# yanglei18/SGV3D

Hardware: AMD Instinct MI355X
Metric: camera frames/sec at 864x1536->BEV (higher is better)
Workload: dtype f32

## Files before the change

include/sgv3d_hip.h:

```cpp
#ifndef SGV3D_HIP_H
#define SGV3D_HIP_H

#include <stddef.h>
#include <stdint.h>

#ifdef __cplusplus
extern "C" {
#endif

#define SGV3D_OK 0
#define SGV3D_EINVAL (-1)
#define SGV3D_ELAUNCH (-2)
#define SGV3D_ENOSPACE (-3)

const char *sgv3d_last_error(void);
int sgv3d_abi_version(void);


int sgv3d_voxel_pooling_forward(int batch_size, int num_points, int num_channels,
                                int num_voxel_x, int num_voxel_y, int num_voxel_z,
                                const int32_t *geom_xyz, const float *input_features,
                                float *output_features, int32_t *pos_memo, void *stream);
int sgv3d_voxel_pooling_forward_fresh(int batch_size, int num_points, int num_channels,
                                      int num_voxel_x, int num_voxel_y, int num_voxel_z,
// ... 226 lines not shown

int sgv3d_deform_im2col3x3(int batch, int h, int w, int channels, int groups, const float *x,
                           const float *offset, int off_ld, float *col, void *stream);

int sgv3d_head_final_conv(int batch, int h, int w, int num_branches, int hidden_ch, int total_out,
                          const float *hidden, const float *weight, const float *bias,
                          const int32_t *branch_of_out, float *out, void *stream);

size_t sgv3d_centerhead_branches_workspace_bytes(int batch, int h, int w, int total_out);
int sgv3d_centerhead_branches_forward(int batch, int h, int w, int cin, int x_ld, int x_coff, const float *x,
                                      int num_branches, const float *w1_wino, const float *scale1,
                                      const float *bias1, int total_out, const float *w2, const float *bias2,
                                      const int32_t *out_begin, float *out, void *workspace,
                                      size_t workspace_bytes, void *stream);

size_t sgv3d_centerhead_f4_weight_floats(int num_branches);
int sgv3d_centerhead_f4_pack_weight(const float *w1, int num_branches, float *u_packed, void *stream);
int sgv3d_centerhead_branches_forward_f4(int batch, int h, int w, int cin, int x_ld, int x_coff, const float *x,
                                         int num_branches, const float *u_packed, const float *scale1,
                                         const float *bias1, int total_out, const float *w2, const float *bias2,
                                         const int32_t *out_begin, float *out, void *workspace,
                                         size_t workspace_bytes, void *stream);

size_t sgv3d_conv3x3_f4res_weight_floats(int cout, int cin);
int sgv3d_conv3x3_f4res_pack_weight(const float *w, int cout, int cin_real, int cin, float *u_packed, void *stream);
int sgv3d_conv3x3_f4res_forward(const sgv3d_conv_desc *d, const float *x, const float *u_packed, const float *scale,
                                const float *bias, const float *residual, float *y, void *stream);

size_t sgv3d_centerhead_bf16_weight_bytes(int num_branches);
int sgv3d_centerhead_bf16_pack_weight(const float *w1, int num_branches, int cin, void *w1_packed, void *stream);
size_t sgv3d_centerhead_bf16_weight2_bytes(int num_branches);
int sgv3d_centerhead_bf16_pack_weight2(const float *w2, const int32_t *out_begin, int num_branches, void *w2_packed,
                                       void *stream);
int sgv3d_centerhead_branches_forward_bf16(int batch, int h, int w, int cin, int x_ld, int x_coff, const float *x,
                                           int num_branches, const void *w1_packed, const float *scale1,
                                           const float *shift1, int total_out, const void *w2_packed, const float *bias2,
                                           const int32_t *out_begin, float *out, void *stream);

int sgv3d_centerhead_branches_forward_bf16x(int batch, int h, int w, int cin, int x_ld, int x_coff, const void *x_bf16,
                                            int num_branches, const void *w1_packed, const float *scale1,
                                            const float *shift1, int total_out, const void *w2_packed, const float *bias2,
                                            const int32_t *out_begin, float *out, void *stream);

void sgv3d_centerhead_bf16_select_plain(int plain);
void sgv3d_centerhead_bf16_debug_stamps(void *buf);

// ... 480 lines not shown
```

sgv3d_amd/_lib.py:

```python
import ctypes
import os

_HERE = os.path.dirname(os.path.abspath(__file__))
LIB_PATH = os.path.join(_HERE, "csrc", "libsgv3d_hip.so")

c_int, c_void_p, c_size_t, c_ll = ctypes.c_int, ctypes.c_void_p, ctypes.c_size_t, ctypes.c_longlong


class ConvDesc(ctypes.Structure):
    _fields_ = [(n, c_int) for n in (
        "batch", "in_h", "in_w", "cin", "out_h", "out_w", "cout", "kh", "kw", "stride", "pad", "dil",
        "x_ld", "x_coff", "y_ld", "y_coff", "res_ld", "relu", "mode", "deconv_ks", "k_pad", "cout_pad",
        "tile", "x_nchw", "k_order", "split_k")]


class VitAttnDesc(ctypes.Structure):
    _fields_ = [(n, c_int) for n in ("batch", "height", "width", "heads", "head_dim", "win_h", "win_w")]


class SamAttnDesc(ctypes.Structure):
    _fields_ = [(n, c_int) for n in ("batch", "nq", "nk", "heads", "head_dim", "q_ld", "k_ld", "v_ld", "o_ld")] + [("scale", ctypes.c_float)]


CONV_NORMAL, CONV_DECONV, CONV_NCHW_OUT, CONV_GROUP_PLANES = 0, 1, 2, 3
# ... 32 lines not shown
    "sgv3d_lift_bf16": (c_int, [c_int] * 4 + [c_void_p] * 4),
    "sgv3d_conv_pack_geometry": (None, [c_int, c_int, ctypes.POINTER(c_int), ctypes.POINTER(c_int)]),
    "sgv3d_conv_pack_weight": (c_int, [c_void_p] + [c_int] * 7 + [c_void_p, c_int, c_int, c_void_p]),
    "sgv3d_conv2d_workspace_bytes": (c_size_t, [ctypes.POINTER(ConvDesc)]),
    "sgv3d_conv2d_forward": (c_int, [ctypes.POINTER(ConvDesc)] + [c_void_p] * 8 + [c_size_t, c_void_p]),
    "sgv3d_conv2d_forward_bf16": (c_int, [ctypes.POINTER(ConvDesc)] + [c_void_p] * 8 + [c_size_t, c_void_p]),
    "sgv3d_conv2d_forward_bf16io": (c_int, [ctypes.POINTER(ConvDesc)] + [c_void_p] * 8 + [c_size_t, c_void_p, c_int]),
    "sgv3d_conv_weight_to_bf16": (c_int, [c_void_p, c_int, c_int, c_void_p, c_void_p]),
    "sgv3d_conv2d_forward_f32x3": (c_int, [ctypes.POINTER(ConvDesc)] + [c_void_p] * 8 + [c_size_t, c_void_p]),
    "sgv3d_centerhead_branches_workspace_bytes": (c_size_t, [c_int] * 4),
    "sgv3d_centerhead_branches_forward": (c_int, [c_int] * 6 + [c_void_p, c_int] + [c_void_p] * 3 + [c_int] + [c_void_p] * 5
                                          + [c_size_t, c_void_p]),
    "sgv3d_centerhead_bf16_weight_bytes": (c_size_t, [c_int]),
    "sgv3d_centerhead_bf16_pack_weight": (c_int, [c_void_p, c_int, c_int, c_void_p, c_void_p]),
    "sgv3d_centerhead_bf16_weight2_bytes": (c_size_t, [c_int]),
    "sgv3d_centerhead_bf16_pack_weight2": (c_int, [c_void_p, c_void_p, c_int, c_void_p, c_void_p]),
    "sgv3d_centerhead_f4_weight_floats": (c_size_t, [c_int]),
    "sgv3d_centerhead_f4_pack_weight": (c_int, [c_void_p, c_int, c_void_p, c_void_p]),
    "sgv3d_centerhead_branches_forward_f4": (c_int, [c_int] * 6 + [c_void_p, c_int] + [c_void_p] * 3 + [c_int] + [c_void_p] * 5
                                             + [c_size_t, c_void_p]),
    "sgv3d_conv3x3_f4res_weight_floats": (c_size_t, [c_int, c_int]),
    "sgv3d_conv3x3_f4res_pack_weight": (c_int, [c_void_p, c_int, c_int, c_int, c_void_p, c_void_p]),
    "sgv3d_conv3x3_f4res_forward": (c_int, [ctypes.POINTER(ConvDesc)] + [c_void_p] * 7),
    "sgv3d_centerhead_branches_forward_bf16": (c_int, [c_int] * 6 + [c_void_p, c_int] + [c_void_p] * 3 + [c_int] + [c_void_p] * 5),
    "sgv3d_centerhead_branches_forward_bf16x": (c_int, [c_int] * 6 + [c_void_p, c_int] + [c_void_p] * 3 + [c_int] + [c_void_p] * 5),
    "sgv3d_centerhead_bf16_select_plain": (None, [c_int]),
    "sgv3d_centerhead_bf16_debug_stamps": (None, [c_void_p]),
    "sgv3d_scale_channels_bf16": (c_int, [c_int] * 3 + [c_void_p] * 4),
    "sgv3d_global_avgpool_bf16": (c_int, [c_int] * 4 + [c_void_p] * 3 + [c_size_t, c_void_p]),
    "sgv3d_broadcast_channels_bf16": (c_int, [c_int] * 5 + [c_void_p] * 3),
    "sgv3d_upsample_bilinear2x_bf16": (c_int, [c_int] * 4 + [c_void_p] * 3),
    "sgv3d_add_mul_sigmoid_bf16": (c_int, [c_ll] + [c_void_p] * 5),
    "sgv3d_deform_im2col3x3_bf16": (c_int, [c_int] * 5 + [c_void_p] * 2 + [c_int, c_void_p, c_void_p]),
    "sgv3d_conv3x3_patch_bf16_weight_bytes": (c_size_t, [c_int, c_int]),
    "sgv3d_conv3x3_patch_bf16_debug_stamps": (None, [c_void_p]),
    "sgv3d_conv3x3_patch_bf16_pack_weight": (c_int, [c_void_p, c_int, c_int, c_void_p, c_void_p]),
    "sgv3d_conv3x3_patch_bf16_forward": (c_int, [c_int] * 11 + [c_void_p] * 6 + [c_int, c_int, c_void_p, c_size_t, c_void_p]),
    "sgv3d_conv_dw_bf16_weight_bytes": (c_size_t, [c_int] * 4),
    "sgv3d_conv_dw_bf16_pack_weight": (c_int, [c_void_p] + [c_int] * 5 + [c_void_p, c_void_p]),
    "sgv3d_conv_dw_bf16_forward": (c_int, [ctypes.POINTER(ConvDesc)] + [c_void_p] * 7),
    "sgv3d_conv_dw_bf16_workspace_bytes": (c_size_t, [ctypes.POINTER(ConvDesc)]),
    "sgv3d_conv_dw_bf16_forward_splitk": (c_int, [ctypes.POINTER(ConvDesc)] + [c_void_p] * 7 + [c_size_t, c_void_p]),
    "sgv3d_conv_dw_bf16_pair_forward": (c_int, [ctypes.POINTER(ConvDesc)] + [c_void_p] * 4 + [c_int] + [c_void_p] * 4 + [c_int, c_void_p, c_int, c_int, c_int, c_void_p]),
    "sgv3d_conv_winograd_weight_floats": (c_size_t, [c_int, c_int]),
    "sgv3d_conv_winograd_pack_weight": (c_int, [c_void_p, c_int, c_int, c_int, c_void_p, c_void_p]),
    "sgv3d_conv2d_winograd_forward": (c_int, [ctypes.POINTER(ConvDesc)] + [c_void_p] * 8 + [c_size_t, c_void_p]),
# ... 210 lines not shown
```

sgv3d_amd/conv_grad.py:

```python
import ctypes

import torch

from . import _lib, grad_slots, pack_cache
from .hip_ops import ConvDesc, PackedConv, prof, _st

__all__ = ['conv2d_backward_weight', 'conv2d_backward_weight_bf16', 'conv2d_backward_weight_batched', 'conv2d_backward_data', 'zero_insert', 'conv2d', 'conv_transpose2d',
           'multi_conv2d', 'thin_conv3x3_forward_batched', 'thin_conv3x3_backward_batched', 'multi_thin_conv2d', 'sliced_thin_conv2d', 'cat_params', 'thin_conv_eligible']


def _out_hw(h, w, k, stride, pad, dil):
    return ((h + 2 * pad - dil * (k[0] - 1) - 1) // stride + 1, (w + 2 * pad - dil * (k[1] - 1) - 1) // stride + 1)


def _dw_buffer(out, shape, device):
    if out is None:
        return torch.empty(*shape, dtype=torch.float32, device=device)
    assert tuple(out.shape) == tuple(shape) and out.is_contiguous() and out.dtype == torch.float32 and out.device == device
    return out


def conv2d_backward_weight(x, dy, kernel, stride=1, pad=0, dil=1, *, cin=None, cout=None, x_coff=0, y_coff=0, split=0, tile=0, out=None):
    kh, kw = (kernel, kernel) if isinstance(kernel, int) else kernel
    B, H, W, x_ld = (int(v) for v in x.shape)
    _, OH, OW, y_ld = (int(v) for v in dy.shape)
    cin = x_ld - x_coff if cin is None else int(cin)
    cout = y_ld - y_coff if cout is None else int(cout)
    if x.dtype == torch.bfloat16:
# ... 626 lines not shown
```

sgv3d_amd/csrc/head_wino4.hip:

```cpp
#include "conv_common.hpp"

using namespace sgv3d;

namespace sgv3d {
int launch_head_ring_fixup(int batch, int h, int w, int total_out, const float *ring, float *out, hipStream_t st);
}

namespace {

typedef float f32x4 __attribute__((ext_vector_type(4)));

constexpr int H4_POS = 36;
constexpr int H4_V_SLOTS = H4_POS * 16 * 16;
constexpr int H4_V_BYTES = H4_V_SLOTS * 16;
constexpr int H4_RED = 9;
constexpr int H4_RED_BYTES = 4 * 64 * H4_RED * 4;
constexpr int H4_LDS = H4_V_BYTES + H4_RED_BYTES;
constexpr int H4_FRAG = 64 * 16;
constexpr int H4_BRANCH = 4 * H4_POS * H4_FRAG;
constexpr int H4_AHEAD = 9;
constexpr int H4_RING = 68;

struct Head4Args {
    const float *x;
    const float *u;
    const float *scale1, *bias1;
    const float *w2, *bias2;
    const int *out_begin;
// ... 409 lines not shown
    SGV3D_REQUIRE((reinterpret_cast<uintptr_t>(x) & 15) == 0 && (reinterpret_cast<uintptr_t>(u_packed) & 15) == 0 &&
                      (reinterpret_cast<uintptr_t>(w2) & 15) == 0 && (!scale1 || (reinterpret_cast<uintptr_t>(scale1) & 15) == 0) &&
                      (!bias1 || (reinterpret_cast<uintptr_t>(bias1) & 15) == 0),
                  "centerhead_branches_forward_f4: x, u_packed, w2, scale1 and bias1 must be 16-B aligned");
    const size_t need = sgv3d_centerhead_branches_workspace_bytes(batch, h, w, total_out);
    if (!workspace || workspace_bytes < need)
        return fail(SGV3D_ENOSPACE, "centerhead_branches_forward_f4: workspace has %zu bytes, needs %zu", workspace_bytes, need);
    Head4Args a;
    a.x = x; a.u = u_packed; a.scale1 = scale1; a.bias1 = bias1; a.w2 = w2; a.bias2 = bias2; a.out_begin = out_begin;
    a.out = out; a.ring = static_cast<float *>(workspace);
    a.x_ld = x_ld; a.x_coff = x_coff; a.h = h; a.w = w; a.nb = num_branches; a.total_out = total_out;
    a.wb_y = cdiv(h, 16); a.wb_x = cdiv(w, 16);
    a.u_bytes = (unsigned)(sgv3d_centerhead_f4_weight_floats(num_branches) * 4);
    static PerDeviceSize lds_set;
    if (!ensure_dynamic_lds(reinterpret_cast<const void *>(&head_wino4_kernel), (size_t)H4_LDS, lds_set))
        return fail(SGV3D_ELAUNCH, "centerhead_branches_forward_f4: cannot raise the dynamic LDS limit to %d", H4_LDS);
    hipStream_t st = as_stream(stream);
    hipLaunchKernelGGL(head_wino4_kernel, dim3(batch * a.wb_y * a.wb_x), dim3(256), H4_LDS, st, a);
    const int rc = launch_head_ring_fixup(batch, h, w, total_out, a.ring, out, st);
    if (rc != SGV3D_OK) return rc;
    return check_launch("head_wino4_kernel");
}

extern "C" size_t sgv3d_conv3x3_f4res_weight_floats(int cout, int cin) {
    if (cout <= 0 || cin <= 0 || cout % 64 || cin % 64 || (cout != 64 && cin != 64)) return 0;
    return (size_t)(cout / 64) * (cin / 64) * 4 * (H4_BRANCH / 4);
}

extern "C" int sgv3d_conv3x3_f4res_pack_weight(const float *w, int cout, int cin_real, int cin, float *u_packed, void *stream) {
    const long long total = (long long)sgv3d_conv3x3_f4res_weight_floats(cout, cin);
    SGV3D_REQUIRE(w && u_packed && total > 0 && cin_real > 0 && cin_real <= cin,
                  "conv3x3_f4res_pack_weight: needs cout and cin multiples of 64, one of them 64 (got %d, %d / %d real)", cout, cin, cin_real);
    SGV3D_REQUIRE(total * 4 < 0xf0000000LL, "conv3x3_f4res_pack_weight: packed weights larger than 3.75 GiB");
    hipLaunchKernelGGL(h4_pack_kernel, dim3(cdiv(total, 256)), dim3(256), 0, as_stream(stream), w, cout / 64, cin / 64, cin_real, u_packed, total);
    return check_launch("h4_pack_kernel");
}

extern "C" int sgv3d_conv3x3_f4res_forward(const sgv3d_conv_desc *d, const float *x, const float *u_packed, const float *scale,
                                           const float *bias, const float *residual, float *y, void *stream) {
    SGV3D_REQUIRE(d && x && u_packed && y, "conv3x3_f4res_forward: null pointer");
    SGV3D_REQUIRE(d->kh == 3 && d->kw == 3 && d->stride == 1 && d->dil == 1 && d->pad == 1 && d->mode == SGV3D_CONV_NORMAL,
                  "conv3x3_f4res_forward: only 3x3 / stride 1 / dilation 1 / pad 1, NHWC output (got k%dx%d s%d d%d p%d mode %d)", d->kh,
                  d->kw, d->stride, d->dil, d->pad, d->mode);
    SGV3D_REQUIRE(d->batch > 0 && d->in_h > 0 && d->in_w > 0 && d->out_h == d->in_h && d->out_w == d->in_w,
                  "conv3x3_f4res_forward: bad map size");
    SGV3D_REQUIRE(sgv3d_conv3x3_f4res_weight_floats(d->cout, d->cin) > 0,
                  "conv3x3_f4res_forward: needs cin and cout multiples of 64, one of them 64 (got %d -> %d)", d->cin, d->cout);
    SGV3D_REQUIRE((d->x_ld & 3) == 0 && (d->x_coff & 3) == 0 && d->x_ld >= d->x_coff + d->cin && (d->y_ld & 3) == 0 &&
                      (d->y_coff & 3) == 0 && d->y_ld >= d->y_coff + d->cout && (!residual || ((d->res_ld & 3) == 0 && d->res_ld >= d->cout)),
                  "conv3x3_f4res_forward: channel strides / offsets must be multiples of 4 and cover the channels");
    const uintptr_t al = reinterpret_cast<uintptr_t>(x) | reinterpret_cast<uintptr_t>(u_packed) | reinterpret_cast<uintptr_t>(y) |
                         reinterpret_cast<uintptr_t>(scale) | reinterpret_cast<uintptr_t>(bias) | reinterpret_cast<uintptr_t>(residual);
    SGV3D_REQUIRE((al & 15) == 0, "conv3x3_f4res_forward: pointers must be 16-B aligned");
    F4ResArgs a;
    a.x = x; a.u = u_packed; a.scale = scale; a.bias = bias; a.res = residual; a.y = y;
    a.x_ld = d->x_ld; a.x_coff = d->x_coff; a.y_ld = d->y_ld; a.y_coff = d->y_coff; a.res_ld = d->res_ld; a.relu = d->relu;
    a.h = d->in_h; a.w = d->in_w; a.wb_y = cdiv(d->in_h, 16); a.wb_x = cdiv(d->in_w, 16);
    a.n_ct = d->cout / 64; a.n_kc = d->cin / 64;
    a.u_bytes = (unsigned)(sgv3d_conv3x3_f4res_weight_floats(d->cout, d->cin) * 4);
    static PerDeviceSize lds_set;
    if (!ensure_dynamic_lds(reinterpret_cast<const void *>(&conv_f4res_kernel), (size_t)H4_V_BYTES, lds_set))
        return fail(SGV3D_ELAUNCH, "conv3x3_f4res_forward: cannot raise the dynamic LDS limit to %d", H4_V_BYTES);
    hipLaunchKernelGGL(conv_f4res_kernel, dim3(d->batch * a.wb_y * a.wb_x), dim3(256), H4_V_BYTES, as_stream(stream), a);
    return check_launch("conv_f4res_kernel");
}
```

sgv3d_amd/hip_ops.py:

```python
import ctypes
from collections import namedtuple
from functools import partialmethod

import torch

from . import _lib, conv_tiles, pack_cache
from ._lib import ConvDesc, CONV_NORMAL, CONV_DECONV, CONV_NCHW_OUT, CONV_GROUP_PLANES
from .conv_tiles import (TILE_WINO, TILE_WINO_RES, TILE_PATCH, TILE_WINO_HALF, TILE_WINO4, TILE_WINO4_WIDE, TILE_WINO4_NARROW,
                         TILE_WINO4_OCC, TILE_WINO4_G48, TILE_F4RES)


def _st(t):
    return _lib.stream_handle(t.device)


PROFILE = None
AUTOTUNE = not __import__("os").environ.get("SGV3D_NO_AUTOTUNE")
DETERMINISTIC = __import__("os").environ.get("SGV3D_DETERMINISTIC", "0") not in ("", "0")


def deterministic():
    return DETERMINISTIC or torch.are_deterministic_algorithms_enabled()
PROFILE_DETAIL = False
import os as _os
# ... 117 lines not shown
PW_X3_DIMS = {t: (TILES[t].bm, TILES[t].bn) for t in PW_X3_TILES}


def _pw_x3_tiles(gemm_m, gemm_n, nkt=None, mfirst=True, skip=()):
    out = ()
    for t in PW_X3_TILES:
        bm, bn = PW_X3_DIMS[t]
        wgs = -(-gemm_m // bm) * -(-gemm_n // bn)
        if (bm, bn) in skip or (bn == 256 and gemm_n < 256) or (TILES[t].mfirst and not (mfirst and MFIRST and gemm_n > bn)):
            continue
        if (wgs >= 96 or (SPLIT_K and nkt is not None and nkt >= 16)) and (bn >= 128 or gemm_n <= 64 or wgs < 1024):
            out += (t,)
    return out


def _split_factors(policy, nk, wgs):
    if not SPLIT_K:
        return ()
    pol = conv_tiles.SPLIT_POLICY[policy]
    return tuple(s for s in conv_tiles.SPLITS if nk // s >= pol["min_k"] and wgs < pol["max_wgs"] and wgs * s <= pol["max_total"])


F4RES = _os.environ.get("SGV3D_F4RES", "1") != "0"
OCC5_TILES = conv_tiles.select("igemm", occ5=True) + conv_tiles.select("igemm", occ5=True, mfirst=True)
OCC5 = _os.environ.get("SGV3D_OCC5", "1") != "0"
WINO4 = _os.environ.get("SGV3D_WINO4", "1") != "0"
WINO4_MIN_CHANNELS = 128
WINO_HALF = _os.environ.get("SGV3D_WINO_HALF", "1") != "0"
PATCH_BF16 = _os.environ.get("SGV3D_PATCH_BF16", "1") != "0"
DW_TILES = conv_tiles.family("dw_bf16")
DW_DEEP_TILES = conv_tiles.select("dw_bf16", deep=True)
DW_DEEP = _os.environ.get("SGV3D_DW_DEEP", "1") != "0"
DW_NARROW = _os.environ.get("SGV3D_DW_NARROW", "1") != "0"
DW_DEEP_MAX_WGS = int(_os.environ.get("SGV3D_DW_DEEP_MAX_WGS", "768"))
DW_BF16 = _os.environ.get("SGV3D_DW_BF16", "1") != "0"
DW_SPLIT_K = _os.environ.get("SGV3D_DW_SPLITK", "1") != "0"


class prof:
    __slots__ = ("name", "flops", "nbytes", "extra", "e0")

    def __init__(self, name, flops=0.0, nbytes=0.0, extra=None):
        self.name, self.flops, self.nbytes, self.extra, self.e0 = name, flops, nbytes, extra, None

    def __enter__(self):
        if PROFILE is not None:
# ... 229 lines not shown
            _lib.check(rc, f.packer)
        setattr(self, f.attr, buf)
        for k, v in notes.items():
            setattr(self, k, v)
        if self._entry is not None and (before is not None or src.data_ptr() != self._entry.param.data_ptr()):
            self._entry.register(name, buf, lambda pc: pc._form(name))
        return buf

    w = property(lambda self: self._form('w'), doc="weights packed for the implicit-GEMM kernels, [cout_pad, k_pad] f32")
    w_wino = property(lambda self: self._form('w_wino'), doc="Winograd F(2x2,3x3) weights, None when the layer is not covered")

    _bf16_weights = partialmethod(_form, 'w_bf16')
    _dw_weights = partialmethod(_form, 'w_dw')
    _patch_weights = partialmethod(_form, 'w_patch')

    def wino4_ok(self, d=None, gate=None):
        is3x3 = (not self.transposed and self.kh == 3 and self.kw == 3 and self.stride == 1 and self.pad == self.dil)
        wide = min(self.cin, self.cout) >= WINO4_MIN_CHANNELS or (self.cin >= 64 and self.cout >= 1024)
        ok = (WINO4 and WINOGRAD and is3x3 and not MFMA_BF16 and self.cin % 32 == 0 and self.cout % 4 == 0 and wide and gate is None)
        if ok and d is not None:
            ok = ((d.mode == CONV_NORMAL and d.y_ld % 4 == 0 and d.y_coff % 4 == 0) or
                  (d.mode == CONV_GROUP_PLANES and d.deconv_ks % 4 == 0)) and d.x_ld % 4 == 0 and d.x_coff % 4 == 0 and d.res_ld % 4 == 0
        return ok

    def f4res_ok(self, d=None, gate=None, io=0):
        ok = (F4RES and WINO4 and WINOGRAD and not MFMA_BF16 and not MFMA_F32X3 and not self.transposed and self.kh == 3
              and self.kw == 3 and self.stride == 1 and self.pad == 1 and self.dil == 1 and gate is None and io == 0
              and self.cin % 64 == 0 and self.cout % 64 == 0 and (self.cin == 64 or self.cout == 64))
        if ok and d is not None:
            ok = (d.mode == CONV_NORMAL and d.x_ld % 4 == 0 and d.x_coff % 4 == 0 and d.y_ld % 4 == 0 and d.y_coff % 4 == 0
                  and d.res_ld % 4 == 0)
        return ok

    def pw_x3_ok(self, d=None, gate=None, io=0):
        taps = self.kh * self.kw
        shape_ok = ((self.k_order == 1 and self.cin % 32 == 0 and self.cin >= 64 and taps <= 32) or
                    (self.k_order == 0 and self.cin % 4 == 0 and taps <= 64 and taps * self.cin >= 128))
        ok = (PW_X3 and not MFMA_BF16 and not MFMA_F32X3 and not self.transposed and gate is None and io == 0 and shape_ok
              and self.cout % 4 == 0)
        if ok and d is not None:
            ok = (d.mode == CONV_NORMAL and d.x_ld % 4 == 0 and d.x_coff % 4 == 0 and d.y_ld % 4 == 0 and d.y_coff % 4 == 0
                  and d.res_ld % 4 == 0)
        return ok

    def _dw_eligible(self, d, gate=None, io=0):
        return (MFMA_BF16 and not MFMA_F32X3 and DW_BF16 and io == 3 and d.mode in (CONV_NORMAL, CONV_DECONV)
# ... 194 lines not shown
               lib.sgv3d_conv2d_forward_f32x3 if x3 else lib.sgv3d_conv2d_forward)
        return fwd(self._abi(d, T), x.data_ptr(), self.w.data_ptr(), *tail, _lib.ptr(gate), out.data_ptr(), _lib.ptr(ws), nws, _st(x))

    def _launch_winograd(self, lib, T, d, x, tail, gate, out, io, ws, nws):
        if not self.wino_ok:
            raise _lib.SGV3DError("this layer has no Winograd weights (needs 3x3 / stride 1 / pad 1 / cin % 8 == 0)")
        return lib.sgv3d_conv2d_winograd_forward(self._abi(d, T), x.data_ptr(), self.w_wino.data_ptr(), *tail, _lib.ptr(gate),
                                                 out.data_ptr(), _lib.ptr(ws), nws, _st(x))

    def _launch_winograd4(self, lib, T, d, x, tail, gate, out, io, ws, nws):
        if not self.wino4_ok(d, gate) or d.split_k > 1:
            raise _lib.SGV3DError("F(4x4) Winograd covers f32 3x3 / stride 1 / pad 1 layers with cin % 32 == 0, cout % 4 == 0, "
                                  "NHWC output, no gate, no split-K")
        u = self._form(T.form)
        a = self._abi(d, T, self.cin, self.wino4_x3_cout_pad) if T.x3 else self._abi(d, T, *self.wino4_geom)
        nws4 = lib.sgv3d_conv2d_winograd4_workspace_bytes(a)
        ws4 = torch.empty(nws4, dtype=torch.uint8, device=x.device)
        return lib.sgv3d_conv2d_winograd4_forward(a, x.data_ptr(), u.data_ptr(), *tail, out.data_ptr(), ws4.data_ptr(), nws4, _st(x))

    def _launch_f4res(self, lib, T, d, x, tail, gate, out, io, ws, nws):
        if not self.f4res_ok(d, gate, io) or d.split_k > 1 or x.dtype != torch.float32:
            raise _lib.SGV3DError("the resident F(4x4) kernel covers f32 3x3 / stride 1 / pad 1 layers with 64 input channels "
                                  "(cout % 64 == 0) or 64 output channels (cin % 64 == 0), NHWC output, no gate, no split-K")
        return lib.sgv3d_conv3x3_f4res_forward(self._abi(d, T), x.data_ptr(), self._form(T.form).data_ptr(), *tail, out.data_ptr(), _st(x))

    def _launch_x3(self, lib, T, d, x, tail, gate, out, io, ws, nws):
        if not self.pw_x3_ok(d, gate, io) or x.dtype != torch.float32:
            raise _lib.SGV3DError("the implicit-GEMM f32x3 kernel covers f32 layers with at most 32 taps, cin % 32 == 0 (>= 64), cout % 4 == 0, "
                                  "NHWC output, no gate")
        u = self._form(T.form)
        return lib.sgv3d_conv2d_x3_forward(self._abi(d, T, d.k_pad, self.pw_x3_cout_pad), x.data_ptr(), u.data_ptr(), *tail, out.data_ptr(),
                                           _lib.ptr(ws), nws, _st(x))

    def _launch_patch_bf16(self, lib, T, d, x, tail, gate, out, io, ws, nws):
        if not self._patch_eligible(d, gate):
            raise _lib.SGV3DError("the bf16 patch kernel covers 3x3 / stride 1 / pad 1 layers with cin % 32 == 0 in bf16 mode")
        return lib.sgv3d_conv3x3_patch_bf16_forward(d.batch, d.in_h, d.in_w, self.cin, self.cout, d.x_ld, d.x_coff, d.y_ld,
                                                    d.y_coff, d.res_ld, d.relu, x.data_ptr(), self._patch_weights().data_ptr(),
                                                    *tail, out.data_ptr(), int(io), int(d.split_k), _lib.ptr(ws), nws, _st(x))

    def _launch_dw_bf16(self, lib, T, d, x, tail, gate, out, io, ws, nws):
        if not self._dw_eligible(d, gate, io) or (d.split_k > 1 and d.mode != CONV_NORMAL):
            raise _lib.SGV3DError("the bf16 direct-weight kernel covers layers with cin % 32 == 0, cout % 8 == 0 and bf16 tensors in "
                                  "and out (NHWC), no gate; split-K in NORMAL mode only")
        if d.split_k > 1:
            nws = lib.sgv3d_conv_dw_bf16_workspace_bytes(ctypes.byref(d))
# ... 185 lines not shown
            st.wait_stream(cur)
            with torch.cuda.stream(st):
                results[i] = t()
        results[0] = thunks[0]()
    finally:
        for st in mine:
            cur.wait_stream(st)
        _BRANCH_TOP[key] = top
    return results


_GRAPH_SPLIT_HOOK = None


def graph_split_point(tag):
    if _GRAPH_SPLIT_HOOK is not None:
        _GRAPH_SPLIT_HOOK(tag)


def switch_state():
    g = globals()
    return tuple(g.get(k) for k in ("AUTOTUNE", "SPLIT_K", "WINOGRAD", "FUSED_HEAD", "HEAD_PATH", "MFMA_BF16", "BF16_ACTIVATIONS",
                                    "MFMA_F32X3", "MFIRST", "WINO4", "WINO_HALF", "PATCH_BF16", "DW_BF16", "DW_DEEP", "DW_NARROW",
                                    "DW_SPLIT_K", "DW_DEEP_MAX_WGS", "PAIR_BF16", "TUNE_STREAMS", "PARALLEL_BRANCHES", "F4RES", "OCC5", "WINO4_G48", "DCN_FUSED", "WINO4_X3", "PW_X3",
                                    "DCN_FUSED_BF16", "DCN_FUSED_TRAIN", "TRAIN_BF16_STORAGE", "SHORTCUT_X3", "DECONV_X3", "VIT_BF16", "STEM_FUSED"))


def conv_pair_eligible(a, b, x, residual=None):
    return (MFMA_BF16 and not MFMA_F32X3 and DW_BF16 and PAIR_BF16 and x.dtype == torch.bfloat16 and not a.transposed and not b.transposed
            and a.cout == 256 and a.cin % 32 == 0 and int(x.shape[-1]) % 8 == 0 and b.cin == 256 and b.kh == 1 and b.kw == 1
            and b.stride == 1 and b.pad == 0 and b.cout % 256 == 0 and (residual is None or residual.dtype == torch.bfloat16))


def conv_pair_bf16(a, b, x, residual=None, out=None):
    B, H, W, x_ld = (int(v) for v in x.shape)
    oh, ow = a.out_hw(H, W)
    if out is None:
        out = torch.empty(B, oh, ow, b.cout, dtype=torch.bfloat16, device=x.device)
    d = ConvDesc()
    d.batch, d.in_h, d.in_w, d.cin = B, H, W, a.cin
    d.out_h, d.out_w, d.cout = oh, ow, a.cout
    d.kh, d.kw, d.stride, d.pad, d.dil = a.kh, a.kw, a.stride, a.pad, a.dil
    d.x_ld, d.x_coff, d.y_ld, d.y_coff = x_ld, 0, a.cout, 0
    d.relu, d.mode, d.split_k = (1 if a.relu else 0), CONV_NORMAL, 1
    flops = 2.0 * B * oh * ow * (a.cout_real * a.cin_real * a.kh * a.kw + b.cout_real * b.cin_real)
    name = "conv_dw_bf16_pair"
    if PROFILE_DETAIL:
# ... 708 lines not shown
```

Before: 296.7.

## Add bf16x3 MFMA variant of resident F(4x4) Winograd 3x3 conv

Adds a new kernel for the resident F(4x4,3x3) Winograd convolution. It splits transformed inputs and weights into three bf16 parts and accumulates six bf16 MFMA products in f32, emulating f32 precision on the matrix cores instead of using the f32 path. Packed weights now hold both the f32 and the x3 forms. A mode switch, set from Python and defaulting to cin==64 layers only, routes eligible layers to the new kernel. This trades extra MFMA work and larger weight storage for higher matrix-core throughput, at the risk of slight numeric differences.

Result: no change. 296.9, median of 2 (+0.1%).

```diff
diff --git a/include/sgv3d_hip.h b/include/sgv3d_hip.h
--- a/include/sgv3d_hip.h
+++ b/include/sgv3d_hip.h
@@ -272,6 +272,7 @@
                                          const int32_t *out_begin, float *out, void *workspace,
                                          size_t workspace_bytes, void *stream);
 
+void sgv3d_conv3x3_f4res_set_x3(int mode);
 size_t sgv3d_conv3x3_f4res_weight_floats(int cout, int cin);
 int sgv3d_conv3x3_f4res_pack_weight(const float *w, int cout, int cin_real, int cin, float *u_packed, void *stream);
 int sgv3d_conv3x3_f4res_forward(const sgv3d_conv_desc *d, const float *x, const float *u_packed, const float *scale,
diff --git a/sgv3d_amd/_lib.py b/sgv3d_amd/_lib.py
--- a/sgv3d_amd/_lib.py
+++ b/sgv3d_amd/_lib.py
@@ -78,6 +78,7 @@
     "sgv3d_conv3x3_f4res_weight_floats": (c_size_t, [c_int, c_int]),
     "sgv3d_conv3x3_f4res_pack_weight": (c_int, [c_void_p, c_int, c_int, c_int, c_void_p, c_void_p]),
     "sgv3d_conv3x3_f4res_forward": (c_int, [ctypes.POINTER(ConvDesc)] + [c_void_p] * 7),
+    "sgv3d_conv3x3_f4res_set_x3": (None, [c_int]),
     "sgv3d_centerhead_branches_forward_bf16": (c_int, [c_int] * 6 + [c_void_p, c_int] + [c_void_p] * 3 + [c_int] + [c_void_p] * 5),
     "sgv3d_centerhead_branches_forward_bf16x": (c_int, [c_int] * 6 + [c_void_p, c_int] + [c_void_p] * 3 + [c_int] + [c_void_p] * 5),
     "sgv3d_centerhead_bf16_select_plain": (None, [c_int]),
diff --git a/sgv3d_amd/conv_grad.py b/sgv3d_amd/conv_grad.py
--- a/sgv3d_amd/conv_grad.py
+++ b/sgv3d_amd/conv_grad.py
@@ -3,7 +3,12 @@
 import torch
 
 from . import _lib, grad_slots, pack_cache
-from .hip_ops import ConvDesc, PackedConv, prof, _st
+from . import hip_ops
+from .hip_ops import ConvDesc, prof, _st
+
+
+class PackedConv(hip_ops.PackedConv):
+    f4res_x3 = False
 
 __all__ = ['conv2d_backward_weight', 'conv2d_backward_weight_bf16', 'conv2d_backward_weight_batched', 'conv2d_backward_data', 'zero_insert', 'conv2d', 'conv_transpose2d',
            'multi_conv2d', 'thin_conv3x3_forward_batched', 'thin_conv3x3_backward_batched', 'multi_thin_conv2d', 'sliced_thin_conv2d', 'cat_params', 'thin_conv_eligible']
diff --git a/sgv3d_amd/csrc/conv_f4res_x3.hip b/sgv3d_amd/csrc/conv_f4res_x3.hip
--- /dev/null
+++ b/sgv3d_amd/csrc/conv_f4res_x3.hip
@@ -0,0 +1,285 @@
+#include "conv_common.hpp"
+
+using namespace sgv3d;
+
+namespace {
+
+typedef float f32x4 __attribute__((ext_vector_type(4)));
+typedef float f32x2 __attribute__((ext_vector_type(2)));
+typedef __bf16 bf16x8 __attribute__((ext_vector_type(8)));
+typedef __bf16 bf16x2 __attribute__((ext_vector_type(2)));
+
+constexpr int RX_POS = 18;
+constexpr int RX_FRAG = 1024;
+constexpr int RX_V_BYTES = RX_POS * 3 * RX_FRAG;
+constexpr int RX_STEP = RX_POS * 3 * RX_FRAG;
+constexpr int RX_AHEAD = 3;
+
+struct F4ResX3Args {
+    const float *x, *scale, *bias, *res;
+    const void *u;
+    float *y;
+    int x_ld, x_coff, y_ld, y_coff, res_ld, relu, h, w, wb_y, wb_x;
+    int n_ct, n_kc;
+    unsigned u_bytes;
+};
+
+template <typename T>
+__device__ __forceinline__ void rx_bt(T &d0, T &d1, T &d2, T &d3, T &d4, T &d5) {
+    const T a = d4 - 4.f * d2, b = d3 - 4.f * d1;
+    const T c = d4 - d2, e = d3 - d1;
+    const T t0 = 4.f * d0 + (d4 - 5.f * d2);
+    const T t5 = 4.f * d1 + (d5 - 5.f * d3);
+    d0 = t0;
+    d1 = a + b;
+    d2 = a - b;
+    d3 = c + 2.f * e;
+    d4 = c - 2.f * e;
+    d5 = t5;
+}
+__device__ __forceinline__ void rx_at(float m0, float m1, float m2, float m3, float m4, float m5, float &y0, float &y1,
+                                      float &y2, float &y3) {
+    const float p = m1 + m2, q = m1 - m2, r = m3 + m4, s = m3 - m4;
+    y0 = (m0 + p) + r;
+    y1 = fmaf(2.f, s, q);
+    y2 = fmaf(4.f, r, p);
+    y3 = fmaf(8.f, s, q) + m5;
+}
+
+__device__ __forceinline__ bf16x8 rx_wload(__amdgpu_buffer_rsrc_t rsrc, unsigned voff, unsigned soff) {
+    return __builtin_bit_cast(bf16x8, __builtin_amdgcn_raw_buffer_load_b128(rsrc, voff, soff, 0));
+}
+
+#define RX_SB() __builtin_amdgcn_sched_barrier(0)
+#define RX_BARRIER() asm volatile("s_waitcnt lgkmcnt(0)\n\ts_barrier" ::: "memory")
+#define RX_MFMA(A, B, C) C = __builtin_amdgcn_mfma_f32_16x16x32_bf16(A, B, C, 0, 0, 0)
+
+template <int HALF>
+__device__ __forceinline__ void rx_transform(f32x2 (&v)[3][6], __amdgpu_buffer_rsrc_t xr, unsigned xoff, unsigned soff, unsigned xs,
+                                             int h, int w, int iy0, int ix0) {
+    f32x2 d[6][6];
+#pragma unroll
+    for (int i = 0; i < 6; ++i) {
+        const bool rok = (unsigned)(iy0 + i) < (unsigned)h;
+        const unsigned ro = xoff + (unsigned)(i * w) * xs;
+#pragma unroll
+        for (int jj = 0; jj < 6; ++jj) {
+            const bool ok = rok & ((unsigned)(ix0 + jj) < (unsigned)w);
+            d[i][jj] = __builtin_bit_cast(f32x2, __builtin_amdgcn_raw_buffer_load_b64(xr, ok ? ro + (unsigned)jj * xs : 0xffffffffu, soff, 0));
+        }
+        RX_SB();
+    }
+#pragma unroll
+    for (int jj = 0; jj < 6; ++jj) rx_bt(d[0][jj], d[1][jj], d[2][jj], d[3][jj], d[4][jj], d[5][jj]);
+#pragma unroll
+    for (int i = 0; i < 3; ++i) {
+        rx_bt(d[3 * HALF + i][0], d[3 * HALF + i][1], d[3 * HALF + i][2], d[3 * HALF + i][3], d[3 * HALF + i][4], d[3 * HALF + i][5]);
+#pragma unroll
+        for (int jj = 0; jj < 6; ++jj) v[i][jj] = d[3 * HALF + i][jj];
+    }
+}
+
+__device__ __forceinline__ void rx_split_store(unsigned char *dst, const f32x2 x) {
+    const bf16x2 hi = __builtin_convertvector(x, bf16x2);
+    const f32x2 r1 = x - __builtin_convertvector(hi, f32x2);
+    const bf16x2 mid = __builtin_convertvector(r1, bf16x2);
+    const f32x2 r2 = r1 - __builtin_convertvector(mid, f32x2);
+    const bf16x2 lo = __builtin_convertvector(r2, bf16x2);
+    *reinterpret_cast<bf16x2 *>(dst) = hi;
+    *reinterpret_cast<bf16x2 *>(dst + RX_FRAG) = mid;
+    *reinterpret_cast<bf16x2 *>(dst + 2 * RX_FRAG) = lo;
+}
+
+template <int HALF>
+__device__ __forceinline__ void rx_step(f32x4 (&acc)[36], unsigned char *smem, unsigned vw, unsigned vr, __amdgpu_buffer_rsrc_t xr,
+                                        unsigned xoff, unsigned soff, unsigned xs, int h, int w, int iy0, int ix0, __amdgpu_buffer_rsrc_t rsrc, unsigned w_lane, unsigned w_off) {
+    bf16x8 wf[RX_AHEAD][3];
+    {
+        asm volatile("" : "+v"(xoff), "+v"(iy0), "+v"(ix0));
+        f32x2 v[3][6];
+        rx_transform<HALF>(v, xr, xoff, soff, xs, h, w, iy0, ix0);
+        RX_SB();
+#pragma unroll
+        for (int r = 0; r < RX_AHEAD; ++r)
+#pragma unroll
+            for (int s = 0; s < 3; ++s) wf[r][s] = rx_wload(rsrc, w_lane, w_off + (unsigned)((r * 3 + s) * RX_FRAG));
+        RX_SB();
+        RX_BARRIER();
+#pragma unroll
+        for (int i = 0; i < 3; ++i)
+#pragma unroll
+            for (int jj = 0; jj < 6; ++jj) rx_split_store(smem + vw + (i * 6 + jj) * 3 * RX_FRAG, v[i][jj]);
+        RX_BARRIER();
+    }
+    const unsigned char *vb = smem + vr;
+    bf16x8 bv[2][3];
+#pragma unroll
+    for (int s = 0; s < 3; ++s) bv[0][s] = *reinterpret_cast<const bf16x8 *>(vb + s * RX_FRAG);
+#pragma unroll
+    for (int p = 0; p < RX_POS; ++p) {
+        RX_SB();
+        if (p + 1 < RX_POS) {
+#pragma unroll
+            for (int s = 0; s < 3; ++s) bv[(p + 1) & 1][s] = *reinterpret_cast<const bf16x8 *>(vb + ((p + 1) * 3 + s) * RX_FRAG);
+        }
+        const bf16x8 u0 = wf[p % RX_AHEAD][0], u1 = wf[p % RX_AHEAD][1], u2 = wf[p % RX_AHEAD][2];
+        if (p + RX_AHEAD < RX_POS) {
+#pragma unroll
+            for (int s = 0; s < 3; ++s)
+                wf[p % RX_AHEAD][s] = rx_wload(rsrc, w_lane, w_off + (unsigned)(((p + RX_AHEAD) * 3 + s) * RX_FRAG));
+        }
+        RX_SB();
+        const bf16x8 *v = bv[p & 1];
+        f32x4 &c = acc[HALF * RX_POS + p];
+        RX_MFMA(u2, v[0], c);
+        RX_MFMA(u0, v[2], c);
+        RX_MFMA(u1, v[1], c);
+        RX_MFMA(u1, v[0], c);
+        RX_MFMA(u0, v[1], c);
+        RX_MFMA(u0, v[0], c);
+        RX_SB();
+    }
+}
+
+__global__ __launch_bounds__(256, 2) void conv_f4res_x3_kernel(const F4ResX3Args a) {
+    __shared__ __attribute__((aligned(16))) unsigned char smem[RX_V_BYTES];
+    const int tid = threadIdx.x;
+    const int lane = tid & 63;
+    const int wave = __builtin_amdgcn_readfirstlane(tid >> 6);
+    const int tm = blockIdx.x;
+    const int bpi = a.wb_y * a.wb_x;
+    const int img = tm / bpi;
+    const int rb = tm - img * bpi;
+    const int by = rb / a.wb_x, bx = rb - by * a.wb_x;
+    const int oy0 = by * 16, ox0 = bx * 16;
+
+    const int jt = tid >> 4, cp = tid & 15;
+    const int iy0 = oy0 + 4 * (jt & 3) - 1, ix0 = ox0 + 4 * (jt >> 2) - 1;
+    const unsigned vw = (unsigned)(jt * 64 + (((cp >> 2) ^ ((-(jt >> 2)) & 3)) << 4) + (cp & 3) * 4);
+    const unsigned xs = (unsigned)a.x_ld * 4u;
+    const __amdgpu_buffer_rsrc_t xr = __builtin_amdgcn_make_buffer_rsrc(
+        const_cast<float *>(a.x + (size_t)img * a.h * a.w * a.x_ld + a.x_coff), 0, (int)((unsigned)(a.h * a.w) * xs - (unsigned)a.x_coff * 4u),
+        0x00020000);
+    const unsigned xoff = (unsigned)(iy0 * a.w + ix0) * xs + (unsigned)cp * 8u;
+    const int g = lane >> 4, j = lane & 15;
+    const unsigned vr = (unsigned)(j * 64 + ((g ^ ((-(j >> 2)) & 3)) << 4));
+
+    const __amdgpu_buffer_rsrc_t rsrc = __builtin_amdgcn_make_buffer_rsrc(const_cast<void *>(a.u), 0, (int)a.u_bytes, 0x00020000);
+    const unsigned w_lane = (unsigned)lane * 16u;
+    unsigned w_off = (unsigned)wave * (unsigned)(a.n_ct * a.n_kc) * (unsigned)(4 * RX_STEP);
+
+    for (int ct = 0; ct < a.n_ct; ++ct) {
+        f32x4 acc[36];
+#pragma unroll
+        for (int p = 0; p < 36; ++p) acc[p] = f32x4{0.f, 0.f, 0.f, 0.f};
+#pragma unroll 1
+        for (int c32 = 0; c32 < 2 * a.n_kc; ++c32) {
+            rx_step<0>(acc, smem, vw, vr, xr, xoff, (unsigned)c32 * 128u, xs, a.h, a.w, iy0, ix0, rsrc, w_lane, w_off);
+            rx_step<1>(acc, smem, vw, vr, xr, xoff, (unsigned)c32 * 128u, xs, a.h, a.w, iy0, ix0, rsrc, w_lane, w_off + (unsigned)RX_STEP);
+            w_off += (unsigned)(2 * RX_STEP);
+        }
+        int tid_ = tid, oy0_ = oy0, ox0_ = ox0;
+        asm volatile("" : "+v"(tid_), "+s"(oy0_), "+s"(ox0_));
+        const int lane_ = tid_ & 63, g_ = lane_ >> 4, j_ = lane_ & 15;
+        const int py0 = oy0_ + 4 * (j_ & 3), px0 = ox0_ + 4 * (j_ >> 2);
+        const int co0 = ct * 64 + wave * 16 + 4 * g_;
+        const f32x4 sc = a.scale ? *reinterpret_cast<const f32x4 *>(a.scale + co0) : f32x4{1.f, 1.f, 1.f, 1.f};
+        const f32x4 sh = a.bias ? *reinterpret_cast<const f32x4 *>(a.bias + co0) : f32x4{0.f, 0.f, 0.f, 0.f};
+        float hd[4][16];
+#pragma unroll
+        for (int r = 0; r < 4; ++r) {
+            float t[4][6];
+#pragma unroll
+            for (int jj = 0; jj < 6; ++jj)
+                rx_at(acc[jj][r], acc[6 + jj][r], acc[12 + jj][r], acc[18 + jj][r], acc[24 + jj][r], acc[30 + jj][r], t[0][jj],
+                      t[1][jj], t[2][jj], t[3][jj]);
+#pragma unroll
+            for (int u = 0; u < 4; ++u)
+                rx_at(t[u][0], t[u][1], t[u][2], t[u][3], t[u][4], t[u][5], hd[r][u * 4], hd[r][u * 4 + 1], hd[r][u * 4 + 2],
+                      hd[r][u * 4 + 3]);
+        }
+        const float floor_ = a.relu ? 0.f : -__builtin_inff();
+#pragma unroll
+        for (int u = 0; u < 4; ++u)
+#pragma unroll
+            for (int v = 0; v < 4; ++v) {
+                const int Y = py0 + u, X = px0 + v;
+                if (Y < a.h && X < a.w) {
+                    const size_t pix = ((size_t)img * a.h + Y) * a.w + X;
+                    f32x4 o = f32x4{hd[0][u * 4 + v], hd[1][u * 4 + v], hd[2][u * 4 + v], hd[3][u * 4 + v]} * sc + sh;
+                    if (a.res) o += *reinterpret_cast<const f32x4 *>(a.res + pix * a.res_ld + co0);
+                    o = f32x4{fmaxf(o.x, floor_), fmaxf(o.y, floor_), fmaxf(o.z, floor_), fmaxf(o.w, floor_)};
+                    *reinterpret_cast<f32x4 *>(a.y + pix * a.y_ld + a.y_coff + co0) = o;
+                }
+            }
+    }
+}
+
+__global__ void rx_pack_kernel(const float *__restrict__ w, int n_ct, int n_kc, int cin_real, __bf16 *__restrict__ dst, long long total) {
+    const long long i = (long long)blockIdx.x * blockDim.x + threadIdx.x;
+    if (i >= total) return;
+    const int e = (int)(i & 7), lane = (int)((i >> 3) & 63);
+    long long r = i >> 9;
+    const int p = (int)(r % 36);
+    r /= 36;
+    const int hf = (int)(r & 1);
+    r >>= 1;
+    const int kc = (int)(r % n_kc);
+    r /= n_kc;
+    const int ct = (int)(r % n_ct), chunk = (int)(r / n_ct);
+    const int co = ct * 64 + chunk * 16 + (lane & 15), ci = kc * 64 + 32 * hf + 8 * (lane >> 4) + e;
+    double u = 0.0;
+    if (ci < cin_real) {
+        const float *gsrc = w + ((size_t)co * cin_real + ci) * 9;
+        const double G[6][3] = {{0.25, 0, 0},           {-1. / 6, -1. / 6, -1. / 6}, {-1. / 6, 1. / 6, -1. / 6},
+                                {1. / 24, 1. / 12, 1. / 6}, {1. / 24, -1. / 12, 1. / 6}, {0, 0, 1}};
+        const int pi = p / 6, pj = p - pi * 6;
+        double gmax = 0.0;
+        for (int y = 0; y < 3; ++y)
+            for (int x = 0; x < 3; ++x) {
+                u += G[pi][y] * (double)gsrc[y * 3 + x] * G[pj][x];
+                gmax = fmax(gmax, fabs((double)gsrc[y * 3 + x]));
+            }
+        if (fabs(u) < gmax * 0x1p-40) u = 0.0;
+    }
+    const float v = (float)u;
+    const __bf16 hi = (__bf16)v;
+    const float r1 = v - (float)hi;
+    const __bf16 mid = (__bf16)r1;
+    const __bf16 lo = (__bf16)(r1 - (float)mid);
+    __bf16 *q = dst + (i >> 9) * 1536 + (i & 511);
+    q[0] = hi;
+    q[512] = mid;
+    q[1024] = lo;
+}
+
+}
+
+namespace sgv3d {
+
+size_t conv_f4res_x3_weight_bytes(int cout, int cin) { return (size_t)(cout / 64) * (cin / 64) * 4 * (4 * RX_STEP); }
+
+int conv_f4res_x3_pack(const float *w, int cout, int cin_real, int cin, void *u3, hipStream_t st) {
+    const long long total = (long long)(conv_f4res_x3_weight_bytes(cout, cin) / 6);
+    hipLaunchKernelGGL(rx_pack_kernel, dim3(cdiv(total, 256)), dim3(256), 0, st, w, cout / 64, cin / 64, cin_real,
+                       static_cast<__bf16 *>(u3), total);
+    return check_launch("rx_pack_kernel");
+}
+
+int conv_f4res_x3_launch(const sgv3d_conv_desc *d, const float *x, const void *u3, const float *scale, const float *bias,
+                         const float *residual, float *y, hipStream_t st) {
+    const size_t ub = conv_f4res_x3_weight_bytes(d->cout, d->cin);
+    SGV3D_REQUIRE(ub < 0xf0000000ULL, "conv3x3_f4res_forward: packed weights larger than 3.75 GiB");
+    SGV3D_REQUIRE((long long)d->in_h * d->in_w * d->x_ld * 4 < 0xf0000000LL,
+                  "conv3x3_f4res_forward: the f32x3 form reads an image through 32-bit offsets (one image larger than 3.75 GiB)");
+    F4ResX3Args a;
+    a.x = x; a.u = u3; a.scale = scale; a.bias = bias; a.res = residual; a.y = y;
+    a.x_ld = d->x_ld; a.x_coff = d->x_coff; a.y_ld = d->y_ld; a.y_coff = d->y_coff; a.res_ld = d->res_ld; a.relu = d->relu;
+    a.h = d->in_h; a.w = d->in_w; a.wb_y = cdiv(d->in_h, 16); a.wb_x = cdiv(d->in_w, 16);
+    a.n_ct = d->cout / 64; a.n_kc = d->cin / 64;
+    a.u_bytes = (unsigned)ub;
+    hipLaunchKernelGGL(conv_f4res_x3_kernel, dim3(d->batch * a.wb_y * a.wb_x), dim3(256), 0, st, a);
+    return check_launch("conv_f4res_x3_kernel");
+}
+
+}
diff --git a/sgv3d_amd/csrc/head_wino4.hip b/sgv3d_amd/csrc/head_wino4.hip
--- a/sgv3d_amd/csrc/head_wino4.hip
+++ b/sgv3d_amd/csrc/head_wino4.hip
@@ -1,9 +1,15 @@
+#include <atomic>
+
 #include "conv_common.hpp"
 
 using namespace sgv3d;
 
 namespace sgv3d {
 int launch_head_ring_fixup(int batch, int h, int w, int total_out, const float *ring, float *out, hipStream_t st);
+size_t conv_f4res_x3_weight_bytes(int cout, int cin);
+int conv_f4res_x3_pack(const float *w, int cout, int cin_real, int cin, void *u3, hipStream_t st);
+int conv_f4res_x3_launch(const sgv3d_conv_desc *d, const float *x, const void *u3, const float *scale, const float *bias,
+                         const float *residual, float *y, hipStream_t st);
 }
 
 namespace {
@@ -459,9 +465,17 @@
     return check_launch("head_wino4_kernel");
 }
 
-extern "C" size_t sgv3d_conv3x3_f4res_weight_floats(int cout, int cin) {
+static size_t f4res_f32_floats(int cout, int cin) {
     if (cout <= 0 || cin <= 0 || cout % 64 || cin % 64 || (cout != 64 && cin != 64)) return 0;
     return (size_t)(cout / 64) * (cin / 64) * 4 * (H4_BRANCH / 4);
+}
+
+static std::atomic<int> g_f4res_x3{1};
+extern "C" void sgv3d_conv3x3_f4res_set_x3(int mode) { g_f4res_x3.store(mode < 0 ? 0 : mode > 2 ? 2 : mode, std::memory_order_relaxed); }
+
+extern "C" size_t sgv3d_conv3x3_f4res_weight_floats(int cout, int cin) {
+    const size_t f32 = f4res_f32_floats(cout, cin);
+    return f32 ? f32 + conv_f4res_x3_weight_bytes(cout, cin) / 4 : 0;
 }
 
 extern "C" int sgv3d_conv3x3_f4res_pack_weight(const float *w, int cout, int cin_real, int cin, float *u_packed, void *stream) {
@@ -469,8 +483,11 @@
     SGV3D_REQUIRE(w && u_packed && total > 0 && cin_real > 0 && cin_real <= cin,
                   "conv3x3_f4res_pack_weight: needs cout and cin multiples of 64, one of them 64 (got %d, %d / %d real)", cout, cin, cin_real);
     SGV3D_REQUIRE(total * 4 < 0xf0000000LL, "conv3x3_f4res_pack_weight: packed weights larger than 3.75 GiB");
-    hipLaunchKernelGGL(h4_pack_kernel, dim3(cdiv(total, 256)), dim3(256), 0, as_stream(stream), w, cout / 64, cin / 64, cin_real, u_packed, total);
-    return check_launch("h4_pack_kernel");
+    const long long f32 = (long long)f4res_f32_floats(cout, cin);
+    hipLaunchKernelGGL(h4_pack_kernel, dim3(cdiv(f32, 256)), dim3(256), 0, as_stream(stream), w, cout / 64, cin / 64, cin_real, u_packed, f32);
+    const int rc = check_launch("h4_pack_kernel");
+    if (rc != SGV3D_OK) return rc;
+    return conv_f4res_x3_pack(w, cout, cin_real, cin, u_packed + f32, as_stream(stream));
 }
 
 extern "C" int sgv3d_conv3x3_f4res_forward(const sgv3d_conv_desc *d, const float *x, const float *u_packed, const float *scale,
@@ -489,12 +506,15 @@
     const uintptr_t al = reinterpret_cast<uintptr_t>(x) | reinterpret_cast<uintptr_t>(u_packed) | reinterpret_cast<uintptr_t>(y) |
                          reinterpret_cast<uintptr_t>(scale) | reinterpret_cast<uintptr_t>(bias) | reinterpret_cast<uintptr_t>(residual);
     SGV3D_REQUIRE((al & 15) == 0, "conv3x3_f4res_forward: pointers must be 16-B aligned");
+    const int x3_mode = g_f4res_x3.load(std::memory_order_relaxed);
+    if (x3_mode == 2 || (x3_mode == 1 && d->cin == 64))
+        return conv_f4res_x3_launch(d, x, u_packed + f4res_f32_floats(d->cout, d->cin), scale, bias, residual, y, as_stream(stream));
     F4ResArgs a;
     a.x = x; a.u = u_packed; a.scale = scale; a.bias = bias; a.res = residual; a.y = y;
     a.x_ld = d->x_ld; a.x_coff = d->x_coff; a.y_ld = d->y_ld; a.y_coff = d->y_coff; a.res_ld = d->res_ld; a.relu = d->relu;
     a.h = d->in_h; a.w = d->in_w; a.wb_y = cdiv(d->in_h, 16); a.wb_x = cdiv(d->in_w, 16);
     a.n_ct = d->cout / 64; a.n_kc = d->cin / 64;
-    a.u_bytes = (unsigned)(sgv3d_conv3x3_f4res_weight_floats(d->cout, d->cin) * 4);
+    a.u_bytes = (unsigned)(f4res_f32_floats(d->cout, d->cin) * 4);
     static PerDeviceSize lds_set;
     if (!ensure_dynamic_lds(reinterpret_cast<const void *>(&conv_f4res_kernel), (size_t)H4_V_BYTES, lds_set))
         return fail(SGV3D_ELAUNCH, "conv3x3_f4res_forward: cannot raise the dynamic LDS limit to %d", H4_V_BYTES);
diff --git a/sgv3d_amd/hip_ops.py b/sgv3d_amd/hip_ops.py
--- a/sgv3d_amd/hip_ops.py
+++ b/sgv3d_amd/hip_ops.py
@@ -163,6 +163,16 @@
 
 
 F4RES = _os.environ.get("SGV3D_F4RES", "1") != "0"
+F4RES_X3 = {"0": False, "all": "all"}.get(_os.environ.get("SGV3D_F4RES_X3", "1"), True)
+_F4RES_X3_LIB = {}
+
+
+def f4res_lib_mode(lib, mode=None):
+    rec = _F4RES_X3_LIB.setdefault(id(lib), [lib, 1])
+    if mode is not None and mode != rec[1]:
+        lib.sgv3d_conv3x3_f4res_set_x3(mode)
+        rec[1] = mode
+    return rec[1]
 OCC5_TILES = conv_tiles.select("igemm", occ5=True) + conv_tiles.select("igemm", occ5=True, mfirst=True)
 OCC5 = _os.environ.get("SGV3D_OCC5", "1") != "0"
 WINO4 = _os.environ.get("SGV3D_WINO4", "1") != "0"
@@ -438,6 +448,15 @@
             ok = ((d.mode == CONV_NORMAL and d.y_ld % 4 == 0 and d.y_coff % 4 == 0) or
                   (d.mode == CONV_GROUP_PLANES and d.deconv_ks % 4 == 0)) and d.x_ld % 4 == 0 and d.x_coff % 4 == 0 and d.res_ld % 4 == 0
         return ok
+
+    f4res_x3 = True
+
+    def f4res_x3_mode(self):
+        return 0 if not (F4RES_X3 and WINO4_X3 and self.f4res_x3) or MFMA_BF16 else 2 if F4RES_X3 == "all" else 1
+
+    def f4res_x3_on(self):
+        mode = self.f4res_x3_mode()
+        return mode == 2 or (mode == 1 and self.cin == 64)
 
     def f4res_ok(self, d=None, gate=None, io=0):
         ok = (F4RES and WINO4 and WINOGRAD and not MFMA_BF16 and not MFMA_F32X3 and not self.transposed and self.kh == 3
@@ -678,6 +697,7 @@
         if not self.f4res_ok(d, gate, io) or d.split_k > 1 or x.dtype != torch.float32:
             raise _lib.SGV3DError("the resident F(4x4) kernel covers f32 3x3 / stride 1 / pad 1 layers with 64 input channels "
                                   "(cout % 64 == 0) or 64 output channels (cin % 64 == 0), NHWC output, no gate, no split-K")
+        f4res_lib_mode(lib, self.f4res_x3_mode())
         return lib.sgv3d_conv3x3_f4res_forward(self._abi(d, T), x.data_ptr(), self._form(T.form).data_ptr(), *tail, out.data_ptr(), _st(x))
 
     def _launch_x3(self, lib, T, d, x, tail, gate, out, io, ws, nws):
@@ -909,7 +929,7 @@
     g = globals()
     return tuple(g.get(k) for k in ("AUTOTUNE", "SPLIT_K", "WINOGRAD", "FUSED_HEAD", "HEAD_PATH", "MFMA_BF16", "BF16_ACTIVATIONS",
                                     "MFMA_F32X3", "MFIRST", "WINO4", "WINO_HALF", "PATCH_BF16", "DW_BF16", "DW_DEEP", "DW_NARROW",
-                                    "DW_SPLIT_K", "DW_DEEP_MAX_WGS", "PAIR_BF16", "TUNE_STREAMS", "PARALLEL_BRANCHES", "F4RES", "OCC5", "WINO4_G48", "DCN_FUSED", "WINO4_X3", "PW_X3",
+                                    "DW_SPLIT_K", "DW_DEEP_MAX_WGS", "PAIR_BF16", "TUNE_STREAMS", "PARALLEL_BRANCHES", "F4RES", "F4RES_X3", "OCC5", "WINO4_G48", "DCN_FUSED", "WINO4_X3", "PW_X3",
                                     "DCN_FUSED_BF16", "DCN_FUSED_TRAIN", "TRAIN_BF16_STORAGE", "SHORTCUT_X3", "DECONV_X3", "VIT_BF16", "STEM_FUSED"))
 
 
```
